# fischer-hub/panGNN

Measured on NVIDIA B200. Metric: train_edges_per_s, higher is better.
Workload: dtype f32

## Files before the change

include/pangnn_b200.h:

```cpp
#ifndef PANGNN_B200_H
#define PANGNN_B200_H

#include <stddef.h>
#include <stdint.h>

#ifdef __cplusplus
extern "C" {
#endif

#define PANGNN_ABI_VERSION 4

#define PANGNN_OK 0
#define PANGNN_EINVAL (-1)
#define PANGNN_EWORKSPACE (-2)
#define PANGNN_ECUDA (-3)

#define PANGNN_ACT_NONE 0
#define PANGNN_ACT_ELU 1

int pangnn_abi_version(void);
const char *pangnn_last_error(void);
const char *pangnn_source_digest(void);

size_t pangnn_sort_pairs_workspace_bytes(int64_t n);
// ... 25 lines not shown
                          const float *w, const float *dis, int32_t num_nodes, int rows_are_dst,
                          float *val, void *stream);

int pangnn_gcn_aggregate(const int64_t *rowptr, const int32_t *col, const float *val, const float *x,
                         int64_t ldx, int32_t num_rows, int32_t feat, const float *bias, int act,
                         float *y, int64_t ldy, void *stream);

int pangnn_act_bwd_bias(const float *dy, const float *y, int64_t num_rows, int32_t feat, int act,
                        float *g, float *dbias , void *ws, size_t ws_bytes,
                        void *stream);
size_t pangnn_act_bwd_bias_workspace_bytes(int64_t num_rows, int32_t feat);

size_t pangnn_gemm_tn_workspace_bytes(int64_t num_rows, int32_t m, int32_t k);
int pangnn_gemm_tn(const float *a, int64_t lda, const float *b, int64_t ldb, int64_t num_rows,
                   int32_t m, int32_t k, float *c, void *ws, size_t ws_bytes, void *stream);

int pangnn_node_linear(const float *x, int64_t ldx, int64_t num_rows, int32_t k, const float *w,
                       int64_t ldw, int w_is_kn, int32_t n, const float *bias, int act, float *y,
                       int64_t ldy, void *stream);
int pangnn_node_linear_push(const float *x, int64_t ldx, int64_t num_rows, int32_t k, const float *w,
                            int64_t ldw, int w_is_kn, int32_t n, const float *bias, int act, float *y,
                            int64_t ldy, const int32_t *push_slot0, float *peer_y0, int64_t lo0, int64_t hi0,
                            const int32_t *push_slot1, float *peer_y1, int64_t lo1, int64_t hi1, void *stream);

size_t pangnn_hits_sort_unique_workspace_bytes(int64_t num_hits);
int pangnn_hits_sort_unique(const int32_t *q, const int32_t *t, const double *bits, int64_t num_hits,
                            int32_t num_nodes, int32_t *q_out, int32_t *t_out, double *bits_out,
                            uint32_t *count , void *ws, size_t ws_bytes, void *stream);
size_t pangnn_hits_normalize_workspace_bytes(int64_t num_hits);
int pangnn_hits_normalize(const int32_t *q, const int32_t *t, const double *bits, int64_t num_hits,
                          const int32_t *genome_of, const int32_t *group_of, double temp, double eps,
                          double pseudo, int drop_trivial, int32_t *src, int32_t *dst, float *w,
                          float *y, uint32_t *count , void *ws, size_t ws_bytes,
                          void *stream);

int pangnn_rows_gather_copy(const float *src, int64_t ld_src, const int32_t *idx, int64_t n, int32_t feat, float *dst,
                            int64_t ld_dst, void *stream);
int pangnn_rows_scatter_add(const float *src, int64_t ld_src, const int32_t *idx, int64_t n, int32_t feat, float *dst,
                            int64_t ld_dst, void *stream);

#define PANGNN_GRAD_REDUCE_MAX_TENSORS 32
#define PANGNN_GRAD_REDUCE_MAX_RANKS 8
int64_t pangnn_grad_bucket_floats(const int64_t *numels, int32_t count);
int pangnn_grad_push(float *const *grads, const int64_t *numels, int32_t count, float *bucket, int64_t half_floats,
                     int32_t *const *peer_signals, int32_t world, int32_t rank, int32_t *ctrl, void *stream);
int pangnn_grad_reduce(float *const *grads, const int64_t *numels, int32_t count, const float *const *peer_buckets,
// ... 123 lines not shown
```

pangnn_b200/_abi.py:

```python
import ctypes as C
import os

from . import build as _build

_c_p = C.c_void_p
_i64, _i32, _sz, _f32, _f64, _int = C.c_int64, C.c_int32, C.c_size_t, C.c_float, C.c_double, C.c_int

SIGNATURES = {
    "pangnn_abi_version": (_int, []),
    "pangnn_last_error": (C.c_char_p, []),
    "pangnn_source_digest": (C.c_char_p, []),
    "pangnn_sort_pairs_workspace_bytes": (_sz, [_i64]),
    "pangnn_sort_pairs_u64": (_int, [_c_p, _c_p, _c_p, _c_p, _i64, _int, _c_p, _sz, _c_p]),
    "pangnn_scan_workspace_bytes": (_sz, [_i64]),
    "pangnn_exclusive_scan_u32": (_int, [_c_p, _c_p, _i64, _c_p, _c_p, _sz, _c_p]),
    "pangnn_csr_build_workspace_bytes": (_sz, [_i64]),
    "pangnn_csr_build": (_int, [_c_p, _i64, _i32, _int, _c_p, _c_p, _c_p, _c_p, _sz, _c_p]),
    "pangnn_gcn_norm": (_int, [_c_p, _c_p, _c_p, _c_p, _i32, _c_p, _c_p, _c_p]),
    "pangnn_gcn_norm_apply": (_int, [_c_p, _c_p, _c_p, _c_p, _c_p, _i32, _int, _c_p, _c_p]),
    "pangnn_gcn_aggregate": (_int, [_c_p, _c_p, _c_p, _c_p, _i64, _i32, _i32, _c_p, _int, _c_p, _i64, _c_p]),
    "pangnn_act_bwd_bias": (_int, [_c_p, _c_p, _i64, _i32, _int, _c_p, _c_p, _c_p, _sz, _c_p]),
    "pangnn_act_bwd_bias_workspace_bytes": (_sz, [_i64, _i32]),
    "pangnn_gemm_tn_workspace_bytes": (_sz, [_i64, _i32, _i32]),
    "pangnn_gemm_tn": (_int, [_c_p, _i64, _c_p, _i64, _i64, _i32, _i32, _c_p, _c_p, _sz, _c_p]),
    "pangnn_node_linear": (_int, [_c_p, _i64, _i64, _i32, _c_p, _i64, _int, _i32, _c_p, _int, _c_p, _i64, _c_p]),
    "pangnn_node_linear_push": (_int, [_c_p, _i64, _i64, _i32, _c_p, _i64, _int, _i32, _c_p, _int, _c_p, _i64,
                                       _c_p, _c_p, _i64, _i64, _c_p, _c_p, _i64, _i64, _c_p]),
    "pangnn_hits_sort_unique_workspace_bytes": (_sz, [_i64]),
    "pangnn_hits_sort_unique": (_int, [_c_p, _c_p, _c_p, _i64, _i32, _c_p, _c_p, _c_p, _c_p, _c_p, _sz, _c_p]),
    "pangnn_hits_normalize_workspace_bytes": (_sz, [_i64]),
    "pangnn_hits_normalize": (_int, [_c_p, _c_p, _c_p, _i64, _c_p, _c_p, _f64, _f64, _f64, _int,
                                     _c_p, _c_p, _c_p, _c_p, _c_p, _c_p, _sz, _c_p]),
    "pangnn_rows_gather_copy": (_int, [_c_p, _i64, _c_p, _i64, _i32, _c_p, _i64, _c_p]),
    "pangnn_rows_scatter_add": (_int, [_c_p, _i64, _c_p, _i64, _i32, _c_p, _i64, _c_p]),
    "pangnn_grad_bucket_floats": (_i64, [_c_p, _i32]),
    "pangnn_grad_push": (_int, [_c_p, _c_p, _i32, _c_p, _i64, _c_p, _i32, _i32, _c_p, _c_p]),
    "pangnn_grad_reduce": (_int, [_c_p, _c_p, _i32, _c_p, _i64, _c_p, _i32, _i32, _c_p, _i64, _c_p]),
    "pangnn_edges_sorted": (_int, [_c_p, _i64, _i32, _c_p, _c_p]),
    "pangnn_csr_from_sorted": (_int, [_c_p, _i64, _i32, _c_p, _c_p, _c_p, _c_p]),
    "pangnn_csr_transpose": (_int, [_c_p, _c_p, _c_p, _i64, _i32, _c_p, _c_p, _c_p, _c_p, _sz, _c_p]),
    "pangnn_csr_merge_band": (_int, [_c_p, _c_p, _c_p, _i64, _i64, _i32, _int, _c_p, _c_p, _c_p, _c_p]),
    "pangnn_csr_spmv2": (_int, [_c_p, _c_p, _c_p, _c_p, _i32, _c_p, _c_p, _c_p]),
    "pangnn_rank1_affine_act": (_int, [_c_p, _c_p, _c_p, _c_p, _c_p, _i64, _i32, _int, _c_p, _i64, _c_p]),
    "pangnn_rank1_bwd_workspace_bytes": (_sz, [_i64, _i32]),
    "pangnn_rank1_bwd": (_int, [_c_p, _c_p, _c_p, _c_p, _i64, _i32, _int, _c_p, _c_p, _sz, _c_p]),
    "pangnn_parse_hits_tsv_workspace_bytes": (_sz, [_i64]),
    "pangnn_tsv_line_index": (_int, [_c_p, _i64, _c_p, _i64, _c_p, _c_p, _sz, _c_p]),
    "pangnn_tsv_parse_hits": (_int, [_c_p, _i64, _c_p, _i64, _i64, _i32, _c_p, _c_p, _i32, _c_p, _c_p, _c_p, _c_p]),
    "pangnn_components_init": (_int, [_c_p, _i32, _c_p]),
    "pangnn_components_round": (_int, [_c_p, _c_p, _c_p, _i64, _c_p, _i32, _c_p, _c_p]),
# ... 65 lines not shown
```

pangnn_b200/csrc/node_linear.cu:

```cuda
#include "common.cuh"
#include "umma.cuh"

namespace pangnn {

namespace {

constexpr int kTileM = 128;
constexpr int kKC = 32;
constexpr int kThreadsNL = 256;
constexpr int kThreadsNLAll = kThreadsNL + 32;
constexpr uint32_t kChunkA = kTileM * 16 + 16;

__device__ __forceinline__ float elu1f(float x) { return x > 0.f ? x : __expf(x) - 1.0f; }

struct NLPush {
    const int32_t *slot0, *slot1;
    float *peer0, *peer1;
    int64_t lo0, hi0, lo1, hi1;
};

template <int N, int K>
struct NLSmem {
    static constexpr uint32_t chunkB = N * 16 + 16;
    static constexpr uint32_t bytesB = (K / 4) * chunkB;
    static constexpr uint32_t bytesA = (kKC / 4) * kChunkA;
    static constexpr uint32_t ringSlot = kTileM * kKC * 4;
    static constexpr uint32_t budget = 227u * 1024u - 2048u;
    static constexpr int stages = ((int64_t)budget - (int64_t)(2 * bytesB + 4 * bytesA + 256) - 8 * 32 * (32 * 4 + 16)) / (int64_t)ringSlot >= 3 ? 2 : 1;
    static constexpr int partC = (budget - (2 * bytesB + 2 * bytesA + 256) - 8 * 32 * (32 * 4 + 16)) / ringSlot >= 3 ? 32 : 16;
    static constexpr uint32_t stageRow = partC * 4 + 16;
    static constexpr uint32_t bytesStage = 8 * 32 * stageRow;
    static constexpr uint32_t fixed = 2 * bytesB + 2 * stages * bytesA + bytesStage + 256;
    static constexpr int ringSlots = ((budget - fixed) / ringSlot) > 6 ? 6 : (int)((budget - fixed) / ringSlot);
    static constexpr uint32_t offBhi = 0, offBlo = bytesB, offA = 2 * bytesB;
    static constexpr uint32_t offStage = (offA + 2 * stages * bytesA + 127) / 128 * 128;
    static constexpr uint32_t offRing = (offStage + bytesStage + 127) / 128 * 128;
    static constexpr uint32_t total = offRing + ringSlots * ringSlot + 64;
    static constexpr int tmemCols = 4 * N;
    static_assert(ringSlots >= 2, "ring too small");
};

__device__ __forceinline__ void cp_async16(uint32_t dst_smem, const void *src) {
    asm volatile("cp.async.cg.shared.global [%0], [%1], 16;" :: "r"(dst_smem), "l"(src) : "memory");
}
__device__ __forceinline__ void cp_async_commit() { asm volatile("cp.async.commit_group;" ::: "memory"); }
template <int NPENDING>
__device__ __forceinline__ void cp_async_wait() { asm volatile("cp.async.wait_group %0;" :: "n"(NPENDING) : "memory"); }

template <int N, int K>
__global__ void __launch_bounds__(kThreadsNLAll, 1)
node_linear_kernel(const float *__restrict__ x, int64_t ldx, int64_t M, const float *__restrict__ w,
                   int64_t ldw, int w_is_kn, const float *__restrict__ bias, int act,
                   float *__restrict__ y, int64_t ldy, const NLPush push) {
    using S = NLSmem<N, K>;
    extern __shared__ __align__(128) uint8_t smem[];
    __shared__ __align__(8) uint64_t bar_stage[2], bar_ready[2], bar_full[2], bar_dfree[2];
    __shared__ uint32_t tmem_base_s;
    const int tid = threadIdx.x, warp = tid >> 5, lane = tid & 31;
    const uint32_t sbase = umma::smem_u32(smem);
    constexpr int NCH = K / kKC;
    constexpr int RS = S::ringSlots;

    if (warp == 0) umma::tmem_alloc(&tmem_base_s, S::tmemCols);
    if (tid == 32) {
        umma::mbar_init(&bar_stage[0], 1);
        umma::mbar_init(&bar_stage[1], 1);
        umma::mbar_init(&bar_full[0], 1);
        umma::mbar_init(&bar_full[1], 1);
        umma::mbar_init(&bar_ready[0], kThreadsNL);
        umma::mbar_init(&bar_ready[1], kThreadsNL);
        umma::mbar_init(&bar_dfree[0], kThreadsNL);
        umma::mbar_init(&bar_dfree[1], kThreadsNL);
        umma::fence_mbar_init();
    }
    for (int idx = tid; idx < N * K; idx += kThreadsNLAll) {
        int n, k;
// ... 12 lines not shown
    const uint32_t tmem_d = tmem_base_s;

    const int64_t num_tiles = (M + kTileM - 1) / kTileM;
    const int64_t my_tiles = blockIdx.x < num_tiles ? (num_tiles - blockIdx.x + gridDim.x - 1) / gridDim.x : 0;
    const int64_t n_items = my_tiles * NCH;
    const int f = tid & 7, rb = tid >> 3;
    constexpr uint32_t idesc = umma::idesc_tf32(kTileM, N, false, false);

    auto issue_item = [&](int64_t it) {
        if (it < n_items) {
            const int64_t tile = blockIdx.x + (it / NCH) * gridDim.x;
            const int c = (int)(it % NCH);
            const uint32_t slot = sbase + S::offRing + (uint32_t)(it % RS) * S::ringSlot;
#pragma unroll
            for (int i = 0; i < 4; ++i) {
                const int r = rb + 32 * i;
                const int64_t row = tile * kTileM + r;
                if (row < M) cp_async16(slot + (uint32_t)r * 128 + (uint32_t)f * 16, x + row * ldx + c * kKC + f * 4);
            }
        }
        cp_async_commit();
    };

    auto epilogue = [&](int64_t t_local) {
        const int64_t tile = blockIdx.x + t_local * gridDim.x;
        const int buf = (int)(t_local & 1);
        umma::mbar_wait(&bar_full[buf], (uint32_t)((t_local >> 1) & 1));
        umma::fence_after_sync();
        const int q = warp & 3, h = warp >> 2;
        constexpr int COLS = N / 2;
        constexpr int PC = S::partC;
        uint8_t *stg = smem + S::offStage + (uint32_t)warp * 32 * S::stageRow;
        const int64_t row0 = tile * kTileM + q * 32;
#pragma unroll
        for (int part = 0; part < COLS / PC; ++part) {
            const int c0 = h * COLS + part * PC;
            float v[PC], vs[PC];
            const uint32_t ta = tmem_d + (uint32_t)(buf * 2 * N) + ((uint32_t)(q * 32) << 16) + (uint32_t)c0;
            umma::tmem_ld<PC>(ta, v);
            umma::tmem_ld<PC>(ta + N, vs);
#pragma unroll
            for (int j = 0; j < PC; ++j) v[j] += vs[j];
#pragma unroll
            for (int j = 0; j < PC; j += 4) {
                float4 o = make_float4(v[j], v[j + 1], v[j + 2], v[j + 3]);
                if (bias) {
                    const float4 b = __ldg(reinterpret_cast<const float4 *>(bias + c0 + j));
                    o.x += b.x; o.y += b.y; o.z += b.z; o.w += b.w;
                }
                if (act == PANGNN_ACT_ELU) { o.x = elu1f(o.x); o.y = elu1f(o.y); o.z = elu1f(o.z); o.w = elu1f(o.w); }
                *reinterpret_cast<float4 *>(stg + (uint32_t)lane * S::stageRow + j * 4) = o;
            }
            __syncwarp();
            constexpr int LPR = PC / 4;
#pragma unroll
            for (int r0 = 0; r0 < 32; r0 += 32 / LPR) {
                const int r = r0 + lane / LPR, fl = lane % LPR;
                const float4 o = *reinterpret_cast<const float4 *>(stg + (uint32_t)r * S::stageRow + fl * 16);
                if (row0 + r < M) {
                    *reinterpret_cast<float4 *>(y + (row0 + r) * ldy + c0 + fl * 4) = o;
                    const int64_t gr = row0 + r;
                    if (push.slot0 && gr >= push.lo0 && gr < push.hi0) {
                        const int32_t ps = __ldg(push.slot0 + gr);
                        if (ps >= 0) *reinterpret_cast<float4 *>(push.peer0 + (int64_t)ps * ldy + c0 + fl * 4) = o;
                    }
                    if (push.slot1 && gr >= push.lo1 && gr < push.hi1) {
                        const int32_t ps = __ldg(push.slot1 + gr);
                        if (ps >= 0) *reinterpret_cast<float4 *>(push.peer1 + (int64_t)ps * ldy + c0 + fl * 4) = o;
                    }
                }
            }
            __syncwarp();
        }
        umma::fence_before_sync();
    };

    constexpr int ST = S::stages;
    if (warp == kThreadsNL / 32) {
#pragma unroll 1
        for (int64_t it = 0; it < n_items; ++it) {
            const int64_t t_local = it / NCH;
            const int c = (int)(it % NCH);
            const int st = (int)(it % ST);
            umma::mbar_wait(&bar_ready[st], (uint32_t)((it / ST) & 1));
            if (c == 0 && t_local >= 2) umma::mbar_wait(&bar_dfree[t_local & 1], (uint32_t)(((t_local >> 1) - 1) & 1));
            if (lane == 0) {
                umma::fence_after_sync();
                const uint32_t offAhi = S::offA + (uint32_t)st * 2 * S::bytesA, offAlo = offAhi + S::bytesA;
                const uint32_t dm = tmem_d + (uint32_t)((t_local & 1) * 2 * N);
                umma::mma_3xtf32<kKC / 8>(dm, dm + N, sbase + offAhi, sbase + offAlo,
                                 sbase + S::offBhi + (uint32_t)c * (kKC / 4) * S::chunkB,
                                 sbase + S::offBlo + (uint32_t)c * (kKC / 4) * S::chunkB,
                                 kChunkA, 128, 2 * kChunkA, S::chunkB, 128, 2 * S::chunkB, idesc, c > 0);
// ... 26 lines not shown
            if (it >= ST) umma::mbar_wait(&bar_stage[st], (uint32_t)(((it - ST) / ST) & 1));
            const uint32_t offAhi = S::offA + (uint32_t)st * 2 * S::bytesA, offAlo = offAhi + S::bytesA;
#pragma unroll
            for (int i = 0; i < 4; ++i) {
                float4 hi, lo;
                umma::split4(raw[i], hi, lo);
                const uint32_t off = (uint32_t)f * kChunkA + (uint32_t)(rb + 32 * i) * 16;
                *reinterpret_cast<float4 *>(smem + offAhi + off) = hi;
                *reinterpret_cast<float4 *>(smem + offAlo + off) = lo;
            }
            umma::fence_async_smem();
            umma::mbar_arrive(&bar_ready[st]);
            if (c == 0 && t_local > 0) {
                epilogue(t_local - 1);
                umma::mbar_arrive(&bar_dfree[(t_local - 1) & 1]);
            }
        }
        if (my_tiles > 0) epilogue(my_tiles - 1);
        cp_async_wait<0>();
    }
    umma::fence_before_sync();
    __syncthreads();
    if (warp == 0) umma::tmem_dealloc(tmem_d, S::tmemCols);
}

template <int N, int K>
int launch_node_linear(const float *x, int64_t ldx, int64_t M, const float *w, int64_t ldw, int w_is_kn,
                       const float *bias, int act, float *y, int64_t ldy, const NLPush &push, cudaStream_t st) {
    using S = NLSmem<N, K>;
    static bool attr_set = false;
    if (!attr_set) {
        int rc = check_cuda(cudaFuncSetAttribute(node_linear_kernel<N, K>, cudaFuncAttributeMaxDynamicSharedMemorySize,
                                                 (int)S::total), "cudaFuncSetAttribute(node_linear)");
        if (rc) return rc;
        attr_set = true;
    }
    const int64_t tiles = (M + kTileM - 1) / kTileM;
    const unsigned grid = (unsigned)(tiles < kNumSMs ? tiles : kNumSMs);
    node_linear_kernel<N, K><<<grid, kThreadsNLAll, S::total, st>>>(x, ldx, M, w, ldw, w_is_kn, bias, act, y, ldy, push);
    PANGNN_CHECK_LAUNCH("node_linear");
    return PANGNN_OK;
}

}
}

using namespace pangnn;

static int node_linear_dispatch(const float *x, int64_t ldx, int64_t num_rows, int32_t k, const float *w, int64_t ldw,
                                int w_is_kn, int32_t n, const float *bias, int act, float *y, int64_t ldy,
                                const NLPush &push, void *stream) {
    PANGNN_REQUIRE(num_rows >= 0, "negative row count");
    if (num_rows == 0) return PANGNN_OK;
    PANGNN_REQUIRE(x && w && y, "null pointer");
    PANGNN_REQUIRE((n == 64 || n == 128) && (k == 64 || k == 128), "n and k must be 64 or 128");
    PANGNN_REQUIRE(ldx % 4 == 0 && ldy % 4 == 0 && ldx >= k && ldy >= n, "bad row stride");
    PANGNN_REQUIRE(ldw >= (w_is_kn ? n : k), "bad weight stride");
    PANGNN_REQUIRE((uintptr_t)x % 16 == 0 && (uintptr_t)y % 16 == 0 && (!bias || (uintptr_t)bias % 16 == 0),
                   "pointers must be 16-byte aligned");
    PANGNN_REQUIRE((!push.slot0 || (push.peer0 && (uintptr_t)push.peer0 % 16 == 0)) &&
                       (!push.slot1 || (push.peer1 && (uintptr_t)push.peer1 % 16 == 0)), "bad push target");
    cudaStream_t st = (cudaStream_t)stream;
    if (n == 64 && k == 64) return launch_node_linear<64, 64>(x, ldx, num_rows, w, ldw, w_is_kn, bias, act, y, ldy, push, st);
    if (n == 128 && k == 64) return launch_node_linear<128, 64>(x, ldx, num_rows, w, ldw, w_is_kn, bias, act, y, ldy, push, st);
    if (n == 64 && k == 128) return launch_node_linear<64, 128>(x, ldx, num_rows, w, ldw, w_is_kn, bias, act, y, ldy, push, st);
    return launch_node_linear<128, 128>(x, ldx, num_rows, w, ldw, w_is_kn, bias, act, y, ldy, push, st);
}

extern "C" int pangnn_node_linear(const float *x, int64_t ldx, int64_t num_rows, int32_t k, const float *w,
                                  int64_t ldw, int w_is_kn, int32_t n, const float *bias, int act, float *y,
                                  int64_t ldy, void *stream) {
    return node_linear_dispatch(x, ldx, num_rows, k, w, ldw, w_is_kn, n, bias, act, y, ldy, NLPush{nullptr, nullptr, nullptr, nullptr, 0, 0, 0, 0},
                                stream);
}

extern "C" int pangnn_node_linear_push(const float *x, int64_t ldx, int64_t num_rows, int32_t k, const float *w,
                                       int64_t ldw, int w_is_kn, int32_t n, const float *bias, int act, float *y,
                                       int64_t ldy, const int32_t *push_slot0, float *peer_y0, int64_t lo0, int64_t hi0,
                                       const int32_t *push_slot1, float *peer_y1, int64_t lo1, int64_t hi1,
                                       void *stream) {
    return node_linear_dispatch(x, ldx, num_rows, k, w, ldw, w_is_kn, n, bias, act, y, ldy,
                                NLPush{push_slot0, push_slot1, peer_y0, peer_y1, lo0, hi0, lo1, hi1}, stream);
}
```

pangnn_b200/gnn.py:

```python
import math

import torch
from torch import nn

from . import ops
from .setup import args


_SIDE_STREAMS = {}

OPERATOR_LAYER = {"kind": "function"}


def set_operator_layer(kind):
    if kind not in ("function", "library"):
        raise ValueError("operator layer is 'function' or 'library'")
    OPERATOR_LAYER["kind"] = kind


def _side_stream(device):
    key = torch.device(device).index
    if key not in _SIDE_STREAMS:
        _SIDE_STREAMS[key] = torch.cuda.Stream(device=device)
    return _SIDE_STREAMS[key]
# ... 28 lines not shown
        super().__init__()
        self.device = device
        node_embedding_dim, hidden_dim = dims
        if categorical_nodes:
            num = dataset if isinstance(dataset, int) else int(getattr(dataset, "num_genes", 0) or len(dataset.x))
            self.embedding = nn.Embedding(num, node_embedding_dim)
        else:
            self.embedding = nn.Linear(1, node_embedding_dim)
        self.conv_in = GCNConv(node_embedding_dim, hidden_dim, add_self_loops=False)
        self.conv_hidden = GCNConv(hidden_dim, hidden_dim, add_self_loops=False)
        self.conv_out = GCNConv(hidden_dim, node_embedding_dim, add_self_loops=False)
        self.linear_out = nn.Linear(hidden_dim, node_embedding_dim)
        self.activation_fct = nn.ELU()
        self.mlp = nn.Sequential(
            nn.Linear(node_embedding_dim * 2 + (1 if args.skip_connections else 0), node_embedding_dim),
            nn.ReLU(),
            nn.Linear(node_embedding_dim, node_embedding_dim),
            nn.ReLU(),
            nn.Linear(node_embedding_dim, 1))
        self.epoch = 0
        self._categorical = bool(categorical_nodes)
        self.fuse_embedding = True

    def embed(self, graph):
        ELU = ops.ACT_ELU
        if (not self._categorical and graph.x.dim() == 2 and graph.x.size(1) == 1 and self.fuse_embedding
                and OPERATOR_LAYER["kind"] == "function"
                and self.conv_in.out_channels % 4 == 0 and self.conv_in.out_channels <= 256):
            ei = graph.union_edge_index if args.union_edge_weights else graph.edge_index
            emb, cin = self.embedding, self.conv_in
            nodes = ops.embed_conv(graph.x, emb.weight, emb.bias, cin.lin.weight, cin.bias, ei, graph.edge_attr, ELU)
            return self._embed_tail(graph, nodes)
        if self._categorical:
            idx = graph.x if graph.x.dtype == torch.long else (
                graph.node_id if hasattr(graph, "node_id") else
                torch.arange(graph.x.size(0), device=graph.x.device))
            node_embeddings = self.embedding(idx)
        elif graph.x.dim() == 2 and graph.x.size(1) == 1:
            node_embeddings = torch.addcmul(self.embedding.bias, graph.x, self.embedding.weight.t())
        else:
            node_embeddings = self.embedding(graph.x)
        ei = graph.union_edge_index if args.union_edge_weights else graph.edge_index
        nodes = self.conv_in(node_embeddings, ei, graph.edge_attr, _act=ELU)
        return self._embed_tail(graph, nodes)

    def _embed_tail(self, graph, nodes):
        ELU = ops.ACT_ELU
        if args.union_edge_weights:
            for _ in range(max(args.neighbours - 2, 1)):
                nodes = self.conv_hidden(nodes, graph.union_edge_index, graph.edge_attr, _act=ELU)
            nodes = self.conv_out(nodes, graph.union_edge_index, None, _act=ELU)
        elif args.base_model:
            nodes = self.activation_fct(self.linear_out(nodes))
        else:
            nodes = self.conv_out(nodes, graph.neighbour_edge_index, None, _act=ELU)
        return nodes

    def _skip(self, graph):
        if not args.skip_connections:
            return None
        return graph.edge_attr[:graph.edge_index.size(1)].contiguous().float()

    def _use_fused_mlp(self, nodes):
        return "mlp" in args.decoder and nodes.size(1) == ops.SCORER_D

    def forward(self, graph):
        nodes = self.embed(graph)
        gs = ops.graph_struct(graph.edge_index, nodes.size(0))
        link_predictions = None
        if "mlp" in args.decoder:
            if self._use_fused_mlp(nodes):
                m = self.mlp
                link_predictions = ops.EdgeScoreFn.apply(
                    nodes, m[0].weight, m[0].bias, m[2].weight, m[2].bias, m[4].weight, m[4].bias,
                    gs, self._skip(graph))
            else:
                src, dst = graph.edge_index[0], graph.edge_index[1]
                parts = (nodes[src], nodes[dst]) + ((self._skip(graph).unsqueeze(1),)
                                                    if args.skip_connections else ())
# ... 53 lines not shown
                    gs = ops.graph_struct(graph.edge_index, n)
                    gs.src, gs.endpoints32
                    gs.built_on(side, main)
                graph.edge_index.record_stream(side)
            wait(*[k for k in ("edge_attr", "x", "y") if k in ready])
            return graph
        wait("edge_index")
        gs = ops.graph_struct(graph.edge_index, n)
        gs.src, gs.endpoints32
        if not args.base_model:
            if getattr(graph, "neighbour_edge_index", None) is None:
                graph.neighbour_edge_index = ops.neighbour_band(n, args.neighbours, graph.edge_index.device)
            wait("neighbour_edge_index")
            ops.graph_struct(graph.neighbour_edge_index, n).src
        wait()
        return graph

    def forward_loss(self, graph, pos_weight):
        if not self._use_fused_mlp_flag():
            logits = self.forward(graph)
            loss = torch.nn.functional.binary_cross_entropy_with_logits(
                logits, graph.y, pos_weight=torch.as_tensor(float(pos_weight), device=logits.device))
            return loss, logits.detach()
        nodes = self.embed(graph)
        gs = ops.graph_struct(graph.edge_index, nodes.size(0))
        m = self.mlp
        if OPERATOR_LAYER["kind"] == "library":
            from . import torch_ops
            return torch_ops.score_edges_bce(nodes, m[0].weight, m[0].bias, m[2].weight, m[2].bias, m[4].weight,
                                             m[4].bias, graph.edge_index, self._skip(graph), graph.y, float(pos_weight))
        return ops.EdgeScoreBCEFn.apply(
            nodes, m[0].weight, m[0].bias, m[2].weight, m[2].bias, m[4].weight, m[4].bias,
            gs, self._skip(graph), graph.y, float(pos_weight))

    def _use_fused_mlp_flag(self):
        return args.decoder == "mlp" and self.mlp[2].weight.size(0) == ops.SCORER_D

    def decode(self, z, edge_index):
        return ops.edge_pair_score(z, ops.graph_struct(edge_index, z.size(0)), 1)

    def cosine_sim(self, z, edge_index):
        return ops.edge_pair_score(z, ops.graph_struct(edge_index, z.size(0)), 0)
```

pangnn_b200/ops.py:

```python
import ctypes as C
from collections import OrderedDict, namedtuple

import torch

from . import _abi

ACT_NONE, ACT_ELU = 0, 1
SCORER_D = 64
NGRADS = 64 * 64 + 64 + 64 + 1 + 64 + 64

LAUNCHES = {"count": 0}


def _p(t):
    return C.c_void_p(t.data_ptr()) if t is not None else C.c_void_p(0)


def _stream():
    return C.c_void_p(torch.cuda.current_stream().cuda_stream)


def _need_cuda(*ts):
    for t in ts:
        if t is not None and not t.is_cuda:
# ... 265 lines not shown
        if act == ACT_ELU:
            torch.nn.functional.elu_(y)
        if out is not None:
            out.copy_(y)
            return out
        return y
    lib = _abi.load()
    M = x.size(0)
    if out is None:
        out = torch.empty(M, n, dtype=torch.float32, device=x.device)
    if push is None:
        _abi.check(lib.pangnn_node_linear(_p(x), x.stride(0), M, k, _p(w), w.stride(0), 1 if w_is_kn else 0, n,
                                          _p(bias), act, _p(out), out.stride(0), _stream()), "node_linear")
    else:
        (s0, p0, lo0, hi0), (s1, p1, lo1, hi1) = (list(push) + [(None, None, 0, 0), (None, None, 0, 0)])[:2]
        for pt in (p0, p1):
            if pt is not None and pt.stride(0) != out.stride(0):
                raise _abi.PangnnError("peer buffers must have the row stride of the output")
        _abi.check(lib.pangnn_node_linear_push(_p(x), x.stride(0), M, k, _p(w), w.stride(0), 1 if w_is_kn else 0, n,
                                               _p(bias), act, _p(out), out.stride(0), _p(s0), _p(p0), lo0, hi0,
                                               _p(s1), _p(p1), lo1, hi1, _stream()), "node_linear_push")
    LAUNCHES["count"] += 1
    return out


class GraphStruct:

    def __init__(self, edge_index, num_nodes):
        self.edge_index = edge_index
        self.num_nodes = num_nodes
        self.num_edges = edge_index.size(1)
        self._src = None
        if self.num_edges > SMALL_CSR_EDGES and edge_index.dtype == torch.int64 and edge_index.dim() == 2:
            self._src = csr_from_sorted(edge_index, num_nodes)
        self._dst = csr_transpose(self._src) if self._src is not None else csr_build(edge_index, num_nodes, by_dst=True)
        self._ends = None
        self._norm = OrderedDict()
        self._ready = None

    def built_on(self, stream, user_stream):
        ev = torch.cuda.Event()
        ev.record(stream)
        self._ready = ev
        for t in (self._dst, self._src):
            if t is not None:
                for a in (t.rowptr, t.col, t.perm):
# ... 181 lines not shown
        lib = _abi.load()
        N, F = a.numel(), weight.size(0)
        w_e1 = w_e.reshape(-1)
        u, v = torch.mv(weight, w_e1), torch.mv(weight, b_e)
        y = torch.empty(N, F, dtype=torch.float32, device=a.device)
        _abi.check(lib.pangnn_rank1_affine_act(_p(a), _p(c), _p(u), _p(v), _p(bias), N, F, act, _p(y), y.stride(0),
                                               _stream()), "rank1_affine_act")
        LAUNCHES["count"] += 1
        ctx.act, ctx.has_bias = act, bias is not None
        ctx.save_for_backward(a, c, y, w_e1, b_e, weight)
        return y

    @staticmethod
    def backward(ctx, dy):
        lib = _abi.load()
        a, c, y, w_e1, b_e, weight = ctx.saved_tensors
        N, F = y.shape
        dy = dy.contiguous()
        sums = torch.empty(3, F, dtype=torch.float32, device=y.device)
        ws = _ws(lib.pangnn_rank1_bwd_workspace_bytes(N, F), y.device)
        _abi.check(lib.pangnn_rank1_bwd(_p(dy), _p(y), _p(a), _p(c), N, F, ctx.act, _p(sums), _p(ws), ws.numel(),
                                        _stream()), "rank1_bwd")
        LAUNCHES["count"] += 2
        db, du, dv = sums[0], sums[1], sums[2]
        dW = torch.addr(torch.outer(du, w_e1), dv, b_e)
        dw_e = torch.mv(weight.t(), du).unsqueeze(1)
        db_e = torch.mv(weight.t(), dv)
        return None, None, dw_e, db_e, dW, (db if ctx.has_bias else None), None


def _rank1_cached(gs, edge_weight, x):
    ent = gs.norm(edge_weight, need_src=False)
    key = ("rank1", x.data_ptr(), x._version)
    ac = ent.get(key)
    if ac is None:
        for k in [k for k in ent if isinstance(k, tuple) and k[0] == "rank1"]:
            del ent[k]
        ac = ent[key] = rank1_vectors(gs.dst, ent["dst"], x) + (x,)
    return ac[0], ac[1]


def embed_conv(x, w_e, b_e, weight, bias, edge_index, edge_weight=None, act=ACT_NONE):
    _need_cuda(x, weight, edge_index)
    if x.requires_grad:
        raise _abi.PangnnError("embed_conv: node features are data, not parameters")
    a, c = _rank1_cached(graph_struct(edge_index, x.size(0)), edge_weight, x)
    return RankOneFn.apply(a, c, w_e, b_e, weight, bias, act)


def gcn_layer(x, weight, bias, edge_index, edge_weight=None, act=ACT_NONE):
    _need_cuda(x, weight, edge_index)
# ... 53 lines not shown
    args, E = _scorer_operands(pq, w1c, b1, w2, b2, w3, b3, gs, skip)
    dev = pq.device
    if da1 is None:
        da1 = torch.empty(E, SCORER_D, dtype=torch.float32, device=dev)
    if grads is None:
        grads = torch.empty(NGRADS, dtype=torch.float32, device=dev)
    if ws is None:
        ws = _ws(lib.pangnn_edge_score_workspace_bytes(E), dev)
    dlogits = None if dlogits is None else dlogits.contiguous()
    y = None if y is None else y.contiguous()
    _abi.check(lib.pangnn_edge_score_bwd(*map(_p, args), E, _p(dlogits), _p(y), float(pos_weight), float(scale),
                                         _p(da1), _p(grads), _p(logits), _p(loss_sum), _p(ws), ws.numel(), _stream()),
               "edge_score_bwd")
    LAUNCHES["count"] += 2 + (loss_sum is not None)
    return da1, grads


def _scorer_common(h, w1, skip):
    if h.size(1) != SCORER_D or w1.size(0) != SCORER_D:
        raise _abi.PangnnError("the fused edge scorer is built for --node_dim 64")
    return split_w1(w1, skip is not None)


def _unpack_scorer_grads(grads, da1, gs, h, wcat, skip, need_h, scale=None):
    D = SCORER_D
    N = h.size(0)
    dpq = torch.empty(N, 2 * D, dtype=torch.float32, device=h.device)
    segment_sum_edges(gs.src, da1, N, dpq[:, :D])
    segment_sum_edges(gs.dst, da1, N, dpq[:, D:])
    dwcat = gemm_tn(dpq, h)
    if scale is not None:
        grads, dwcat, wcat = grads * scale, dwcat * scale, wcat * scale
    g = scorer_grads(grads)
    dw1 = torch.cat((dwcat[:D], dwcat[D:]) + ((g.dw1c.unsqueeze(1),) if skip is not None else ()), dim=1)
    dh = node_linear(dpq, wcat, w_is_kn=True) if need_h else None
    return dh, dw1, g.db1, g.dW2, g.db2, g.dw3, g.db3


class EdgeScoreFn(torch.autograd.Function):

    @staticmethod
    def forward(ctx, h, w1, b1, w2, b2, w3, b3, gs, skip):
        wcat, w1c = _scorer_common(h, w1, skip)
        pq = node_linear(h, wcat)
        logits = edge_score_pq_fwd(pq, w1c, b1, w2, b2, w3, b3, gs, skip)
        ctx.gs, ctx.skip = gs, skip
        ctx.save_for_backward(h, w1, b1, w2, b2, w3, b3, pq)
        return logits

    @staticmethod
    def backward(ctx, dlogits):
        h, w1, b1, w2, b2, w3, b3, pq = ctx.saved_tensors
        gs, skip = ctx.gs, ctx.skip
        wcat, w1c = _scorer_common(h, w1, skip)
        da1, grads = edge_score_train(pq, w1c, b1, w2, b2, w3, b3, gs, skip, dlogits=dlogits)
        return _unpack_scorer_grads(grads, da1, gs, h, wcat, skip, ctx.needs_input_grad[0]) + (None, None)


class EdgeScoreBCEFn(torch.autograd.Function):

    @staticmethod
    def forward(ctx, h, w1, b1, w2, b2, w3, b3, gs, skip, y, pos_weight):
        wcat, w1c = _scorer_common(h, w1, skip)
        E = gs.num_edges
        pq = node_linear(h, wcat)
        logits = torch.empty(E, dtype=torch.float32, device=h.device)
        loss_sum = torch.zeros(1, dtype=torch.float64, device=h.device)
        da1, grads = edge_score_train(pq, w1c, b1, w2, b2, w3, b3, gs, skip, y=y, pos_weight=pos_weight,
                                      scale=1.0 / max(E, 1), logits=logits, loss_sum=loss_sum)
        ctx.gs, ctx.skip = gs, skip
        ctx.save_for_backward(h, wcat, da1, grads)
        ctx.mark_non_differentiable(logits)
        loss = (loss_sum / max(E, 1)).float().squeeze(0)
        return loss, logits

    @staticmethod
    def backward(ctx, dloss, _dlogits):
        h, wcat, da1, grads = ctx.saved_tensors
        out = _unpack_scorer_grads(grads, da1, ctx.gs, h, wcat, ctx.skip, ctx.needs_input_grad[0],
                                   scale=dloss)
        return out + (None, None, None, None)


class EdgePairScoreFn(torch.autograd.Function):

    @staticmethod
    def forward(ctx, h, gs, mode):
        lib = _abi.load()
        src, dst = gs.endpoints32
        h = h.contiguous()
        out = torch.empty(gs.num_edges, dtype=torch.float32, device=h.device)
        _abi.check(lib.pangnn_edge_pair_score(_p(h), h.stride(0), h.size(1), _p(src), _p(dst),
                                              gs.num_edges, mode, _p(out), _stream()), "edge_pair_score")
        LAUNCHES["count"] += 1
        ctx.gs, ctx.mode = gs, mode
        ctx.save_for_backward(h, out)
        return out

    @staticmethod
    def backward(ctx, dz):
        lib = _abi.load()
        h, out = ctx.saved_tensors
        gs = ctx.gs
        N, F = h.shape
# ... 663 lines not shown
```

Baseline: 890.7 million.

## Fuse ELU backward and bias/rank-1 column sums into node_linear epilogue for whole-chain training

Adds an epilogue mode to the tcgen05 node_linear kernel that multiplies the GEMM output by the ELU derivative of the saved activation, writes the gradient, and accumulates per-block column sums (bias grad, or rank-2 sums weighted by a and c for the first layer). A reduction over blocks then finishes the sums. A new NodeChainBCEFn runs the embedding, conv chain, scorer and loss as one autograd function whose backward uses these fused kernels. The aim is to cut separate activation-backward, bias-reduction and rank-1 backward passes and the autograd overhead between layers. The cost is more register pressure in the epilogue and extra loads of x inside it.

```diff
diff --git a/include/pangnn_b200.h b/include/pangnn_b200.h
--- a/include/pangnn_b200.h
+++ b/include/pangnn_b200.h
@@ -71,6 +71,10 @@
                             int64_t ldw, int w_is_kn, int32_t n, const float *bias, int act, float *y,
                             int64_t ldy, const int32_t *push_slot0, float *peer_y0, int64_t lo0, int64_t hi0,
                             const int32_t *push_slot1, float *peer_y1, int64_t lo1, int64_t hi1, void *stream);
+size_t pangnn_node_linear_elu_bwd_workspace_bytes(int64_t num_rows, int32_t n);
+int pangnn_node_linear_elu_bwd(const float *dh, int64_t ldh, int64_t num_rows, int32_t k, const float *w,
+                               int64_t ldw, int32_t n, const float *x, int64_t ldx, const float *a, const float *c,
+                               float *g, int64_t ldg, float *sums, void *ws, size_t ws_bytes, void *stream);
 
 size_t pangnn_hits_sort_unique_workspace_bytes(int64_t num_hits);
 int pangnn_hits_sort_unique(const int32_t *q, const int32_t *t, const double *bits, int64_t num_hits,
diff --git a/pangnn_b200/_abi.py b/pangnn_b200/_abi.py
--- a/pangnn_b200/_abi.py
+++ b/pangnn_b200/_abi.py
@@ -26,6 +26,9 @@
     "pangnn_node_linear": (_int, [_c_p, _i64, _i64, _i32, _c_p, _i64, _int, _i32, _c_p, _int, _c_p, _i64, _c_p]),
     "pangnn_node_linear_push": (_int, [_c_p, _i64, _i64, _i32, _c_p, _i64, _int, _i32, _c_p, _int, _c_p, _i64,
                                        _c_p, _c_p, _i64, _i64, _c_p, _c_p, _i64, _i64, _c_p]),
+    "pangnn_node_linear_elu_bwd_workspace_bytes": (_sz, [_i64, _i32]),
+    "pangnn_node_linear_elu_bwd": (_int, [_c_p, _i64, _i64, _i32, _c_p, _i64, _i32, _c_p, _i64, _c_p, _c_p, _c_p,
+                                          _i64, _c_p, _c_p, _sz, _c_p]),
     "pangnn_hits_sort_unique_workspace_bytes": (_sz, [_i64]),
     "pangnn_hits_sort_unique": (_int, [_c_p, _c_p, _c_p, _i64, _i32, _c_p, _c_p, _c_p, _c_p, _c_p, _sz, _c_p]),
     "pangnn_hits_normalize_workspace_bytes": (_sz, [_i64]),
diff --git a/pangnn_b200/csrc/node_linear.cu b/pangnn_b200/csrc/node_linear.cu
--- a/pangnn_b200/csrc/node_linear.cu
+++ b/pangnn_b200/csrc/node_linear.cu
@@ -2,6 +2,9 @@
 #include "umma.cuh"
 
 namespace pangnn {
+
+int reduce_partials(const float *partial, int64_t nblocks, int32_t width, int32_t stride, float *out,
+                    cudaStream_t st);
 
 namespace {
 
@@ -12,6 +15,26 @@
 constexpr uint32_t kChunkA = kTileM * 16 + 16;
 
 __device__ __forceinline__ float elu1f(float x) { return x > 0.f ? x : __expf(x) - 1.0f; }
+
+constexpr int kEpiStore = 0, kEpiEluBias = 1, kEpiRank2 = 2;
+
+struct NLBwd {
+    const float *x, *a, *c;
+    int64_t ldx;
+    float *partial;
+};
+
+__device__ __forceinline__ float4 elu_grad4(float4 d, const float4 y) {
+    d.x *= y.x > 0.f ? 1.f : y.x + 1.f;
+    d.y *= y.y > 0.f ? 1.f : y.y + 1.f;
+    d.z *= y.z > 0.f ? 1.f : y.z + 1.f;
+    d.w *= y.w > 0.f ? 1.f : y.w + 1.f;
+    return d;
+}
+__device__ __forceinline__ void add4(float4 &s, const float4 v) { s.x += v.x; s.y += v.y; s.z += v.z; s.w += v.w; }
+__device__ __forceinline__ void fma4(float4 &s, float a, const float4 v) {
+    s.x = fmaf(a, v.x, s.x); s.y = fmaf(a, v.y, s.y); s.z = fmaf(a, v.z, s.z); s.w = fmaf(a, v.w, s.w);
+}
 
 struct NLPush {
     const int32_t *slot0, *slot1;
@@ -47,11 +70,11 @@
 template <int NPENDING>
 __device__ __forceinline__ void cp_async_wait() { asm volatile("cp.async.wait_group %0;" :: "n"(NPENDING) : "memory"); }
 
-template <int N, int K>
+template <int N, int K, int EPI>
 __global__ void __launch_bounds__(kThreadsNLAll, 1)
 node_linear_kernel(const float *__restrict__ x, int64_t ldx, int64_t M, const float *__restrict__ w,
                    int64_t ldw, int w_is_kn, const float *__restrict__ bias, int act,
-                   float *__restrict__ y, int64_t ldy, const NLPush push) {
+                   float *__restrict__ y, int64_t ldy, const NLPush push, const NLBwd bwd) {
     using S = NLSmem<N, K>;
     extern __shared__ __align__(128) uint8_t smem[];
     __shared__ __align__(8) uint64_t bar_stage[2], bar_ready[2], bar_full[2], bar_dfree[2];
@@ -110,6 +133,14 @@
         cp_async_commit();
     };
 
+    constexpr int NSUMS = EPI == kEpiRank2 ? 3 : 1;
+    constexpr int NPART = (N / 2) / S::partC;
+    constexpr int LPR = S::partC / 4;
+    constexpr int RPS = 32 / LPR;
+    float4 csum[EPI == kEpiStore ? 1 : NSUMS * NPART];
+#pragma unroll
+    for (int i = 0; i < (EPI == kEpiStore ? 1 : NSUMS * NPART); ++i) csum[i] = make_float4(0.f, 0.f, 0.f, 0.f);
+
     auto epilogue = [&](int64_t t_local) {
         const int64_t tile = blockIdx.x + t_local * gridDim.x;
         const int buf = (int)(t_local & 1);
@@ -123,6 +154,21 @@
 #pragma unroll
         for (int part = 0; part < COLS / PC; ++part) {
             const int c0 = h * COLS + part * PC;
+            constexpr bool kXAhead = EPI == kEpiEluBias || (EPI == kEpiRank2 && N == 128 && K == 128);
+            float4 xb[EPI == kEpiStore ? 1 : 32 / RPS];
+            float av[EPI == kEpiRank2 ? 32 / RPS : 1], cv[EPI == kEpiRank2 ? 32 / RPS : 1];
+            auto load_x = [&](int i) {
+                const int64_t gr = row0 + i * RPS + lane / LPR;
+                xb[i] = gr < M ? ld_stream_f4(bwd.x + gr * bwd.ldx + c0 + (lane % LPR) * 4) : make_float4(0.f, 0.f, 0.f, 0.f);
+                if constexpr (EPI == kEpiRank2) {
+                    av[i] = gr < M ? __ldg(bwd.a + gr) : 0.f;
+                    cv[i] = gr < M ? __ldg(bwd.c + gr) : 0.f;
+                }
+            };
+            if constexpr (kXAhead) {
+#pragma unroll
+                for (int i = 0; i < 32 / RPS; ++i) load_x(i);
+            }
             float v[PC], vs[PC];
             const uint32_t ta = tmem_d + (uint32_t)(buf * 2 * N) + ((uint32_t)(q * 32) << 16) + (uint32_t)c0;
             umma::tmem_ld<PC>(ta, v);
@@ -140,7 +186,23 @@
                 *reinterpret_cast<float4 *>(stg + (uint32_t)lane * S::stageRow + j * 4) = o;
             }
             __syncwarp();
-            constexpr int LPR = PC / 4;
+            if constexpr (EPI != kEpiStore) {
+#pragma unroll
+                for (int i = 0; i < 32 / RPS; ++i) {
+                    const int r = i * RPS + lane / LPR, fl = lane % LPR;
+                    if constexpr (!kXAhead) load_x(i);
+                    if (row0 + r < M) {
+                        const float4 g = elu_grad4(*reinterpret_cast<const float4 *>(stg + (uint32_t)r * S::stageRow + fl * 16), xb[i]);
+                        add4(csum[part], g);
+                        if constexpr (EPI == kEpiRank2) {
+                            fma4(csum[NPART + part], av[i], g);
+                            fma4(csum[2 * NPART + part], cv[i], g);
+                        } else {
+                            *reinterpret_cast<float4 *>(y + (row0 + r) * ldy + c0 + fl * 4) = g;
+                        }
+                    }
+                }
+            } else {
 #pragma unroll
             for (int r0 = 0; r0 < 32; r0 += 32 / LPR) {
                 const int r = r0 + lane / LPR, fl = lane % LPR;
@@ -157,6 +219,7 @@
                         if (ps >= 0) *reinterpret_cast<float4 *>(push.peer1 + (int64_t)ps * ldy + c0 + fl * 4) = o;
                     }
                 }
+            }
             }
             __syncwarp();
         }
@@ -229,22 +292,52 @@
     umma::fence_before_sync();
     __syncthreads();
     if (warp == 0) umma::tmem_dealloc(tmem_d, S::tmemCols);
-}
-
-template <int N, int K>
+    if constexpr (EPI != kEpiStore) {
+        static_assert(4 * NSUMS * N * sizeof(float) <= S::bytesStage, "column-sum reduction overruns the staging area");
+        float *red = reinterpret_cast<float *>(smem + S::offStage);
+        if (warp < kThreadsNL / 32) {
+            const int q = warp & 3, h = warp >> 2;
+#pragma unroll
+            for (int i = 0; i < NSUMS * NPART; ++i) {
+                float4 s = csum[i];
+#pragma unroll
+                for (int off = LPR; off < 32; off <<= 1) {
+                    s.x += __shfl_xor_sync(0xffffffffu, s.x, off);
+                    s.y += __shfl_xor_sync(0xffffffffu, s.y, off);
+                    s.z += __shfl_xor_sync(0xffffffffu, s.z, off);
+                    s.w += __shfl_xor_sync(0xffffffffu, s.w, off);
+                }
+                const int k = i / NPART, part = i % NPART;
+                if (lane < LPR)
+                    *reinterpret_cast<float4 *>(red + q * NSUMS * N + k * N + h * (N / 2) + part * S::partC + lane * 4) = s;
+            }
+        }
+        __syncthreads();
+        for (int i = tid; i < NSUMS * N; i += kThreadsNLAll)
+            bwd.partial[(int64_t)blockIdx.x * NSUMS * N + i] =
+                ((red[i] + red[NSUMS * N + i]) + red[2 * NSUMS * N + i]) + red[3 * NSUMS * N + i];
+    }
+}
+
+unsigned node_linear_grid(int64_t M) {
+    const int64_t tiles = (M + kTileM - 1) / kTileM;
+    return (unsigned)(tiles < kNumSMs ? (tiles > 0 ? tiles : 1) : kNumSMs);
+}
+
+template <int N, int K, int EPI>
 int launch_node_linear(const float *x, int64_t ldx, int64_t M, const float *w, int64_t ldw, int w_is_kn,
-                       const float *bias, int act, float *y, int64_t ldy, const NLPush &push, cudaStream_t st) {
+                       const float *bias, int act, float *y, int64_t ldy, const NLPush &push, const NLBwd &bwd,
+                       cudaStream_t st) {
     using S = NLSmem<N, K>;
     static bool attr_set = false;
     if (!attr_set) {
-        int rc = check_cuda(cudaFuncSetAttribute(node_linear_kernel<N, K>, cudaFuncAttributeMaxDynamicSharedMemorySize,
+        int rc = check_cuda(cudaFuncSetAttribute(node_linear_kernel<N, K, EPI>, cudaFuncAttributeMaxDynamicSharedMemorySize,
                                                  (int)S::total), "cudaFuncSetAttribute(node_linear)");
         if (rc) return rc;
         attr_set = true;
     }
-    const int64_t tiles = (M + kTileM - 1) / kTileM;
-    const unsigned grid = (unsigned)(tiles < kNumSMs ? tiles : kNumSMs);
-    node_linear_kernel<N, K><<<grid, kThreadsNLAll, S::total, st>>>(x, ldx, M, w, ldw, w_is_kn, bias, act, y, ldy, push);
+    node_linear_kernel<N, K, EPI><<<node_linear_grid(M), kThreadsNLAll, S::total, st>>>(x, ldx, M, w, ldw, w_is_kn,
+                                                                                       bias, act, y, ldy, push, bwd);
     PANGNN_CHECK_LAUNCH("node_linear");
     return PANGNN_OK;
 }
@@ -268,10 +361,21 @@
     PANGNN_REQUIRE((!push.slot0 || (push.peer0 && (uintptr_t)push.peer0 % 16 == 0)) &&
                        (!push.slot1 || (push.peer1 && (uintptr_t)push.peer1 % 16 == 0)), "bad push target");
     cudaStream_t st = (cudaStream_t)stream;
-    if (n == 64 && k == 64) return launch_node_linear<64, 64>(x, ldx, num_rows, w, ldw, w_is_kn, bias, act, y, ldy, push, st);
-    if (n == 128 && k == 64) return launch_node_linear<128, 64>(x, ldx, num_rows, w, ldw, w_is_kn, bias, act, y, ldy, push, st);
-    if (n == 64 && k == 128) return launch_node_linear<64, 128>(x, ldx, num_rows, w, ldw, w_is_kn, bias, act, y, ldy, push, st);
-    return launch_node_linear<128, 128>(x, ldx, num_rows, w, ldw, w_is_kn, bias, act, y, ldy, push, st);
+    const NLBwd nb{nullptr, nullptr, nullptr, 0, nullptr};
+    if (n == 64 && k == 64) return launch_node_linear<64, 64, kEpiStore>(x, ldx, num_rows, w, ldw, w_is_kn, bias, act, y, ldy, push, nb, st);
+    if (n == 128 && k == 64) return launch_node_linear<128, 64, kEpiStore>(x, ldx, num_rows, w, ldw, w_is_kn, bias, act, y, ldy, push, nb, st);
+    if (n == 64 && k == 128) return launch_node_linear<64, 128, kEpiStore>(x, ldx, num_rows, w, ldw, w_is_kn, bias, act, y, ldy, push, nb, st);
+    return launch_node_linear<128, 128, kEpiStore>(x, ldx, num_rows, w, ldw, w_is_kn, bias, act, y, ldy, push, nb, st);
+}
+
+template <int EPI>
+static int node_linear_bwd_dispatch(const float *dh, int64_t ldh, int64_t num_rows, int32_t k, const float *w,
+                                    int64_t ldw, int32_t n, float *g, int64_t ldg, const NLBwd &bwd, cudaStream_t st) {
+    const NLPush np{nullptr, nullptr, nullptr, nullptr, 0, 0, 0, 0};
+    if (n == 64 && k == 64) return launch_node_linear<64, 64, EPI>(dh, ldh, num_rows, w, ldw, 1, nullptr, PANGNN_ACT_NONE, g, ldg, np, bwd, st);
+    if (n == 128 && k == 64) return launch_node_linear<128, 64, EPI>(dh, ldh, num_rows, w, ldw, 1, nullptr, PANGNN_ACT_NONE, g, ldg, np, bwd, st);
+    if (n == 64 && k == 128) return launch_node_linear<64, 128, EPI>(dh, ldh, num_rows, w, ldw, 1, nullptr, PANGNN_ACT_NONE, g, ldg, np, bwd, st);
+    return launch_node_linear<128, 128, EPI>(dh, ldh, num_rows, w, ldw, 1, nullptr, PANGNN_ACT_NONE, g, ldg, np, bwd, st);
 }
 
 extern "C" int pangnn_node_linear(const float *x, int64_t ldx, int64_t num_rows, int32_t k, const float *w,
@@ -289,3 +393,35 @@
     return node_linear_dispatch(x, ldx, num_rows, k, w, ldw, w_is_kn, n, bias, act, y, ldy,
                                 NLPush{push_slot0, push_slot1, peer_y0, peer_y1, lo0, hi0, lo1, hi1}, stream);
 }
+
+extern "C" size_t pangnn_node_linear_elu_bwd_workspace_bytes(int64_t num_rows, int32_t n) {
+    return (size_t)node_linear_grid(num_rows) * 3 * (size_t)(n > 0 ? n : 0) * sizeof(float) + 256;
+}
+
+extern "C" int pangnn_node_linear_elu_bwd(const float *dh, int64_t ldh, int64_t num_rows, int32_t k, const float *w,
+                                          int64_t ldw, int32_t n, const float *x, int64_t ldx, const float *a,
+                                          const float *c, float *g, int64_t ldg, float *sums, void *ws,
+                                          size_t ws_bytes, void *stream) {
+    PANGNN_REQUIRE(num_rows >= 0, "negative row count");
+    PANGNN_REQUIRE((n == 64 || n == 128) && (k == 64 || k == 128), "n and k must be 64 or 128");
+    PANGNN_REQUIRE(sums && ws, "null pointer");
+    PANGNN_REQUIRE((a == nullptr) == (c == nullptr), "a and c go together");
+    if (ws_bytes < pangnn_node_linear_elu_bwd_workspace_bytes(num_rows, n)) {
+        set_error("node_linear_elu_bwd: workspace too small");
+        return PANGNN_EWORKSPACE;
+    }
+    const int nsums = a ? 3 : 1;
+    cudaStream_t st = (cudaStream_t)stream;
+    if (num_rows == 0) return check_cuda(cudaMemsetAsync(sums, 0, (size_t)nsums * n * sizeof(float), st), "memset");
+    PANGNN_REQUIRE(dh && w && x && (a || g), "null pointer");
+    PANGNN_REQUIRE(ldh % 4 == 0 && ldx % 4 == 0 && ldh >= k && ldx >= n && ldw >= n, "bad row stride");
+    PANGNN_REQUIRE(a || (ldg % 4 == 0 && ldg >= n), "bad row stride");
+    PANGNN_REQUIRE((uintptr_t)dh % 16 == 0 && (uintptr_t)x % 16 == 0 && (a || (uintptr_t)g % 16 == 0),
+                   "pointers must be 16-byte aligned");
+    float *partial = static_cast<float *>(ws);
+    const NLBwd bwd{x, a, c, ldx, partial};
+    const int rc = a ? node_linear_bwd_dispatch<kEpiRank2>(dh, ldh, num_rows, k, w, ldw, n, nullptr, 0, bwd, st)
+                     : node_linear_bwd_dispatch<kEpiEluBias>(dh, ldh, num_rows, k, w, ldw, n, g, ldg, bwd, st);
+    if (rc) return rc;
+    return reduce_partials(partial, node_linear_grid(num_rows), nsums * n, nsums * n, sums, st);
+}
diff --git a/pangnn_b200/gnn.py b/pangnn_b200/gnn.py
--- a/pangnn_b200/gnn.py
+++ b/pangnn_b200/gnn.py
@@ -74,11 +74,14 @@
         self._categorical = bool(categorical_nodes)
         self.fuse_embedding = True
 
+    def _rank2_embedding(self, graph):
+        return (not self._categorical and graph.x.dim() == 2 and graph.x.size(1) == 1 and self.fuse_embedding
+                and OPERATOR_LAYER["kind"] == "function"
+                and self.conv_in.out_channels % 4 == 0 and self.conv_in.out_channels <= 256)
+
     def embed(self, graph):
         ELU = ops.ACT_ELU
-        if (not self._categorical and graph.x.dim() == 2 and graph.x.size(1) == 1 and self.fuse_embedding
-                and OPERATOR_LAYER["kind"] == "function"
-                and self.conv_in.out_channels % 4 == 0 and self.conv_in.out_channels <= 256):
+        if self._rank2_embedding(graph):
             ei = graph.union_edge_index if args.union_edge_weights else graph.edge_index
             emb, cin = self.embedding, self.conv_in
             nodes = ops.embed_conv(graph.x, emb.weight, emb.bias, cin.lin.weight, cin.bias, ei, graph.edge_attr, ELU)
@@ -97,16 +100,30 @@
         return self._embed_tail(graph, nodes)
 
     def _embed_tail(self, graph, nodes):
-        ELU = ops.ACT_ELU
+        convs = self._tail_convs(graph)
+        if convs is None:
+            return self.activation_fct(self.linear_out(nodes))
+        for conv, ei, ew in convs:
+            nodes = conv(nodes, ei, ew, _act=ops.ACT_ELU)
+        return nodes
+
+    def _tail_convs(self, graph):
         if args.union_edge_weights:
-            for _ in range(max(args.neighbours - 2, 1)):
-                nodes = self.conv_hidden(nodes, graph.union_edge_index, graph.edge_attr, _act=ELU)
-            nodes = self.conv_out(nodes, graph.union_edge_index, None, _act=ELU)
-        elif args.base_model:
-            nodes = self.activation_fct(self.linear_out(nodes))
-        else:
-            nodes = self.conv_out(nodes, graph.neighbour_edge_index, None, _act=ELU)
-        return nodes
+            return ((self.conv_hidden, graph.union_edge_index, graph.edge_attr),) * max(args.neighbours - 2, 1) + \
+                ((self.conv_out, graph.union_edge_index, None),)
+        if args.base_model:
+            return None
+        return ((self.conv_out, graph.neighbour_edge_index, None),)
+
+    def _chain_convs(self, graph):
+        convs = self._tail_convs(graph) if self._rank2_embedding(graph) else None
+        if convs is None or self.conv_in.out_channels not in (64, 128):
+            return None
+        for conv, _, _ in convs:
+            i, o = conv.in_channels, conv.out_channels
+            if i not in (64, 128) or o not in (64, 128) or (i < o and i % 4 == 0):
+                return None
+        return convs
 
     def _skip(self, graph):
         if not args.skip_connections:
@@ -206,9 +223,17 @@
             loss = torch.nn.functional.binary_cross_entropy_with_logits(
                 logits, graph.y, pos_weight=torch.as_tensor(float(pos_weight), device=logits.device))
             return loss, logits.detach()
+        m = self.mlp
+        convs = self._chain_convs(graph)
+        if convs is not None:
+            emb, cin = self.embedding, self.conv_in
+            ei = graph.union_edge_index if args.union_edge_weights else graph.edge_index
+            return ops.node_chain_bce(graph.x, ei, graph.edge_attr, emb.weight, emb.bias, cin.lin.weight, cin.bias,
+                                      tuple((cv.lin.weight, cv.bias, e, w) for cv, e, w in convs),
+                                      m[0].weight, m[0].bias, m[2].weight, m[2].bias, m[4].weight, m[4].bias,
+                                      graph.edge_index, self._skip(graph), graph.y, pos_weight)
         nodes = self.embed(graph)
         gs = ops.graph_struct(graph.edge_index, nodes.size(0))
-        m = self.mlp
         if OPERATOR_LAYER["kind"] == "library":
             from . import torch_ops
             return torch_ops.score_edges_bce(nodes, m[0].weight, m[0].bias, m[2].weight, m[2].bias, m[4].weight,
diff --git a/pangnn_b200/ops.py b/pangnn_b200/ops.py
--- a/pangnn_b200/ops.py
+++ b/pangnn_b200/ops.py
@@ -311,6 +311,26 @@
                                                _p(s1), _p(p1), lo1, hi1, _stream()), "node_linear_push")
     LAUNCHES["count"] += 1
     return out
+
+
+def node_linear_elu_bwd(dh, w, x, a=None, c=None):
+    _need_cuda(dh, w, x)
+    k, n = w.shape
+    if not (_tc_shape(dh, n, k) and _tc_shape(x, n, k) and dh.size(1) == k and x.size(1) == n and w.stride(1) == 1):
+        raise _abi.PangnnError("node_linear_elu_bwd: n, k in {64, 128}, dense 16-byte aligned fp32 rows")
+    lib = _abi.load()
+    M = dh.size(0)
+    rank2 = a is not None
+    g = None if rank2 else torch.empty(M, n, dtype=torch.float32, device=dh.device)
+    sums = torch.empty((3, n) if rank2 else (n,), dtype=torch.float32, device=dh.device)
+    if rank2:
+        a, c = a.contiguous(), c.contiguous()
+    ws = _ws(lib.pangnn_node_linear_elu_bwd_workspace_bytes(M, n), dh.device)
+    _abi.check(lib.pangnn_node_linear_elu_bwd(_p(dh), dh.stride(0), M, k, _p(w), w.stride(0), n, _p(x), x.stride(0),
+                                              _p(a), _p(c), _p(g), g.stride(0) if g is not None else 0, _p(sums),
+                                              _p(ws), ws.numel(), _stream()), "node_linear_elu_bwd")
+    LAUNCHES["count"] += 2
+    return g, sums
 
 
 class GraphStruct:
@@ -538,11 +558,14 @@
         _abi.check(lib.pangnn_rank1_bwd(_p(dy), _p(y), _p(a), _p(c), N, F, ctx.act, _p(sums), _p(ws), ws.numel(),
                                         _stream()), "rank1_bwd")
         LAUNCHES["count"] += 2
-        db, du, dv = sums[0], sums[1], sums[2]
-        dW = torch.addr(torch.outer(du, w_e1), dv, b_e)
-        dw_e = torch.mv(weight.t(), du).unsqueeze(1)
-        db_e = torch.mv(weight.t(), dv)
+        db, dw_e, db_e, dW = _rank1_param_grads(sums, w_e1, b_e, weight)
         return None, None, dw_e, db_e, dW, (db if ctx.has_bias else None), None
+
+
+def _rank1_param_grads(sums, w_e1, b_e, weight):
+    db, du, dv = sums[0], sums[1], sums[2]
+    dW = torch.addr(torch.outer(du, w_e1), dv, b_e)
+    return db, torch.mv(weight.t(), du).unsqueeze(1), torch.mv(weight.t(), dv), dW
 
 
 def _rank1_cached(gs, edge_weight, x):
@@ -642,7 +665,7 @@
     return split_w1(w1, skip is not None)
 
 
-def _unpack_scorer_grads(grads, da1, gs, h, wcat, skip, need_h, scale=None):
+def _unpack_scorer_grads(grads, da1, gs, h, wcat, skip, need_h, scale=None, elu_below=False):
     D = SCORER_D
     N = h.size(0)
     dpq = torch.empty(N, 2 * D, dtype=torch.float32, device=h.device)
@@ -653,7 +676,10 @@
         grads, dwcat, wcat = grads * scale, dwcat * scale, wcat * scale
     g = scorer_grads(grads)
     dw1 = torch.cat((dwcat[:D], dwcat[D:]) + ((g.dw1c.unsqueeze(1),) if skip is not None else ()), dim=1)
-    dh = node_linear(dpq, wcat, w_is_kn=True) if need_h else None
+    if elu_below:
+        dh = node_linear_elu_bwd(dpq, wcat, h)
+    else:
+        dh = node_linear(dpq, wcat, w_is_kn=True) if need_h else None
     return dh, dw1, g.db1, g.dW2, g.db2, g.dw3, g.db3
 
 
@@ -700,6 +726,72 @@
         out = _unpack_scorer_grads(grads, da1, ctx.gs, h, wcat, ctx.skip, ctx.needs_input_grad[0],
                                    scale=dloss)
         return out + (None, None, None, None)
+
+
+class NodeChainBCEFn(torch.autograd.Function):
+
+    @staticmethod
+    def forward(ctx, layers, a, c, w_e, b_e, w0, b0, w1, b1, w2, b2, w3, b3, gs, skip, y, pos_weight, *params):
+        lib = _abi.load()
+        N, F = a.numel(), w0.size(0)
+        w_e1 = w_e.reshape(-1)
+        u, v = torch.mv(w0, w_e1), torch.mv(w0, b_e)
+        x = torch.empty(N, F, dtype=torch.float32, device=a.device)
+        _abi.check(lib.pangnn_rank1_affine_act(_p(a), _p(c), _p(u), _p(v), _p(b0), N, F, ACT_ELU, _p(x), x.stride(0),
+                                               _stream()), "rank1_affine_act")
+        LAUNCHES["count"] += 1
+        xs = [x]
+        for (lgs, ew), weight, bias in zip(layers, params[0::2], params[1::2]):
+            ent = lgs.norm(ew, need_src=False)
+            h = node_linear(xs[-1], weight)
+            xs.append(aggregate(lgs, ent, h, True, bias, ACT_ELU))
+        h = xs[-1]
+        wcat, w1c = _scorer_common(h, w1, skip)
+        E = gs.num_edges
+        pq = node_linear(h, wcat)
+        logits = torch.empty(E, dtype=torch.float32, device=h.device)
+        loss_sum = torch.zeros(1, dtype=torch.float64, device=h.device)
+        da1, grads = edge_score_train(pq, w1c, b1, w2, b2, w3, b3, gs, skip, y=y, pos_weight=pos_weight,
+                                      scale=1.0 / max(E, 1), logits=logits, loss_sum=loss_sum)
+        ctx.layers, ctx.gs, ctx.skip = layers, gs, skip
+        ctx.save_for_backward(a, c, w_e1, b_e, w0, wcat, da1, grads, *params[0::2], *xs)
+        ctx.mark_non_differentiable(logits)
+        loss = (loss_sum / max(E, 1)).float().squeeze(0)
+        return loss, logits
+
+    @staticmethod
+    def backward(ctx, dloss, _dlogits):
+        a, c, w_e1, b_e, w0, wcat, da1, grads, *rest = ctx.saved_tensors
+        L = len(ctx.layers)
+        weights, xs = rest[:L], rest[L:]
+        (g, dbias), dw1, db1, dW2, db2, dw3, db3 = _unpack_scorer_grads(
+            grads, da1, ctx.gs, xs[-1], wcat, ctx.skip, True, scale=dloss, elu_below=True)
+        dparams = [None] * (2 * L)
+        for l in reversed(range(L)):
+            lgs, ew = ctx.layers[l]
+            dh = aggregate(lgs, lgs.norm(ew, need_src=True), g, False)
+            dparams[2 * l] = gemm_tn(dh, xs[l])
+            dparams[2 * l + 1] = dbias
+            if l > 0:
+                g, dbias = node_linear_elu_bwd(dh, weights[l], xs[l])
+            else:
+                _, sums = node_linear_elu_bwd(dh, weights[l], xs[l], a, c)
+        db0, dw_e, db_e, dW0 = _rank1_param_grads(sums, w_e1, b_e, w0)
+        return ((None, None, None, dw_e, db_e, dW0, db0, dw1, db1, dW2, db2, dw3, db3, None, None, None, None)
+                + tuple(dparams))
+
+
+def node_chain_bce(x, first_edge_index, first_edge_weight, w_e, b_e, w0, b0, convs, w1, b1, w2, b2, w3, b3,
+                   edge_index, skip, y, pos_weight):
+    _need_cuda(x, w0, first_edge_index)
+    if x.requires_grad:
+        raise _abi.PangnnError("node_chain_bce: node features are data, not parameters")
+    N = x.size(0)
+    a, c = _rank1_cached(graph_struct(first_edge_index, N), first_edge_weight, x)
+    layers = tuple((graph_struct(ei, N), ew) for _, _, ei, ew in convs)
+    params = tuple(t for wt, bs, _, _ in convs for t in (wt, bs))
+    return NodeChainBCEFn.apply(layers, a, c, w_e, b_e, w0, b0, w1, b1, w2, b2, w3, b3, graph_struct(edge_index, N),
+                                skip, y, float(pos_weight), *params)
 
 
 class EdgePairScoreFn(torch.autograd.Function):
```

New measurement: 925.2 million (median of 6 runs). 1.04x the previous value.
